# run-house/kubetorch

Hardware: NVIDIA H100
Metric: parallel_map_arg_plus_result_GBps (higher is better)
Workload: dtype f32

## Files before the change

### kubetorch_b200/csrc/ktb_map.cu

```cuda
#include "ktb_common.cuh"

#include <algorithm>
#include <atomic>

namespace ktb {

extern int g_red_ctas_per_sm;
extern int g_red_loads;
extern int g_red_fold;
extern int g_seg_large;
extern int g_mlp_chunk_rows;
}
extern int g_mlp_stage_ce;
namespace ktb {
extern std::atomic<int> g_host_zero_copy;
}
extern std::atomic<int> g_push_scatter_ctas_per_sm;
extern std::atomic<int> g_push_slice;
namespace ktb {

static std::atomic<int> g_vec_ctas_per_sm{0};
static std::atomic<int> g_tma_ctas_per_sm{1};
static std::atomic<int> g_tma_cfg{0};
static std::atomic<int> g_auto_variant{KTB_VARIANT_VEC};
static std::atomic<int> g_vec_flavor{2};
static std::atomic<int> g_vec_unroll{4};

constexpr int kVecThreads = 256;
constexpr int kVecUnroll = 4;
constexpr int kVecFlavor = 2;

template <int VB, int FL>
__device__ __forceinline__ void ld_vec(const uint8_t* p, uint32_t (&w)[VB / 4]) {
  static_assert(VB == 16, "sm_90 has no wider per-thread global access than 128 bits");
  if constexpr (FL == 1) {
    asm volatile("ld.global.v4.b32 {%0,%1,%2,%3}, [%4];"
                 : "=r"(w[0]), "=r"(w[1]), "=r"(w[2]), "=r"(w[3])
                 : "l"(p)
                 : "memory");
  } else if constexpr (FL == 2 || FL == 3) {
    ldg128_stream(p, w);
  } else {
    ldg128(p, w);
  }
}
template <int VB, int FL>
__device__ __forceinline__ void st_vec(uint8_t* p, const uint32_t (&w)[VB / 4]) {
  static_assert(VB == 16, "sm_90 has no wider per-thread global access than 128 bits");
  if constexpr (FL == 1) {
    asm volatile("st.global.v4.b32 [%0], {%1,%2,%3,%4};" ::"l"(p), "r"(w[0]), "r"(w[1]), "r"(w[2]), "r"(w[3])
                 : "memory");
  } else if constexpr (FL == 2) {
    stg128_stream(p, w);
  } else {
    stg128(p, w);
  }
}

template <int DT, int OP, int VB, int FL = kVecFlavor, int UNROLL = kVecUnroll>
__global__ void __launch_bounds__(kVecThreads)
    map_vec_kernel(const uint8_t* src, uint8_t* dst, size_t n_bytes, MapParams p) {
  constexpr int NW = VB / 4;
  constexpr int kVecUnroll = UNROLL;
  constexpr size_t TILE = (size_t)kVecThreads * kVecUnroll * VB;
  constexpr size_t ROW = (size_t)kVecThreads * VB;
  const size_t n_full = n_bytes / TILE;

  for (size_t t = blockIdx.x; t < n_full; t += gridDim.x) {
    const size_t off = t * TILE + (size_t)threadIdx.x * VB;
    uint32_t w[kVecUnroll][NW];
#pragma unroll
    for (int j = 0; j < kVecUnroll; ++j) ld_vec<VB, FL>(src + off + j * ROW, w[j]);
#pragma unroll
    for (int j = 0; j < kVecUnroll; ++j) {
      apply_words<DT, OP, NW>(w[j], p);
      st_vec<VB, FL>(dst + off + j * ROW, w[j]);
    }
  }

  if (blockIdx.x == (unsigned)(n_full % gridDim.x)) {
    const size_t base = n_full * TILE;
    const size_t n_vec = (n_bytes - base) / VB;
    for (size_t v = threadIdx.x; v < n_vec; v += kVecThreads) {
      uint32_t w[NW];
      ld_vec<VB, FL>(src + base + v * VB, w);
      apply_words<DT, OP, NW>(w, p);
      st_vec<VB, FL>(dst + base + v * VB, w);
    }
    constexpr size_t ES = (DT == KTB_U8) ? 1 : ((DT == KTB_BF16 || DT == KTB_F16) ? 2 : (DT == KTB_I64 ? 8 : 4));
    const size_t tail = base + n_vec * VB;
    const size_t n_tail = (n_bytes - tail) / ES;
    for (size_t e = threadIdx.x; e < n_tail; e += kVecThreads)
      apply_elem<DT, OP>(src + tail + e * ES, dst + tail + e * ES, p);
  }
}

template <int DT, int OP>
__global__ void __launch_bounds__(256)
    map_scalar_kernel(const uint8_t* src, uint8_t* dst, size_t n_elems, MapParams p) {
  constexpr size_t ES = (DT == KTB_U8) ? 1 : ((DT == KTB_BF16 || DT == KTB_F16) ? 2 : (DT == KTB_I64 ? 8 : 4));
  const size_t stride = (size_t)gridDim.x * blockDim.x;
  for (size_t i = (size_t)blockIdx.x * blockDim.x + threadIdx.x; i < n_elems; i += stride)
    apply_elem<DT, OP>(src + i * ES, dst + i * ES, p);
}

template <int DT, int OP, int STAGES, int STAGE_BYTES, int NT>
__global__ void __launch_bounds__(NT)
    map_tma_kernel(const uint8_t* src, uint8_t* dst, size_t n_bytes, MapParams p) {
  extern __shared__ __align__(128) uint8_t smem[];
  uint8_t* buf = smem;
  uint64_t* full = reinterpret_cast<uint64_t*>(smem + (size_t)STAGES * STAGE_BYTES);
  constexpr bool kCompute = !(OP == KTB_OP_IDENTITY || DT == KTB_U8);
// ... 13 lines not shown
#pragma unroll
    for (int s = 0; s < STAGES; ++s) mbar_init(&full[s], 1);
    fence_barrier_init();
    fence_proxy_async_smem();
  }
  __syncthreads();

  if (threadIdx.x == 0) {
    const size_t pre = my_n < (size_t)STAGES ? my_n : (size_t)STAGES;
    for (size_t k = 0; k < pre; ++k) {
      const uint32_t len = tile_len(k);
      mbar_expect_tx(&full[k], len);
      bulk_g2s(buf + k * STAGE_BYTES, src + tile_off(k), len, &full[k]);
    }
  }

  if (kCompute || threadIdx.x == 0) {
    for (size_t k = 0; k < my_n; ++k) {
      const int s = (int)(k % STAGES);
      const uint32_t parity = (uint32_t)((k / STAGES) & 1);
      const uint32_t len = tile_len(k);
      mbar_wait(&full[s], parity);
      if constexpr (kCompute) {
        uint4* tile = reinterpret_cast<uint4*>(buf + (size_t)s * STAGE_BYTES);
        const uint32_t nv = len >> 4;
        for (uint32_t v = threadIdx.x; v < nv; v += NT) {
          uint4 q = tile[v];
          uint32_t w[4] = {q.x, q.y, q.z, q.w};
          apply_words<DT, OP, 4>(w, p);
          tile[v] = make_uint4(w[0], w[1], w[2], w[3]);
        }
        fence_proxy_async_smem();
        __syncthreads();
      }
      if (threadIdx.x == 0) {
        bulk_s2g(dst + tile_off(k), buf + (size_t)s * STAGE_BYTES, len);
        bulk_commit();
        if (k >= 1 && (k - 1 + STAGES) < my_n) {
          bulk_wait_read<1>();
          const size_t kn = k - 1 + STAGES;
          const int sn = (int)((k - 1) % STAGES);
          const uint32_t ln = tile_len(kn);
          mbar_expect_tx(&full[sn], ln);
          bulk_g2s(buf + (size_t)sn * STAGE_BYTES, src + tile_off(kn), ln, &full[sn]);
        }
      }
    }
    if (threadIdx.x == 0) bulk_wait_all<0>();
  }

  if (blockIdx.x == 0) {
    constexpr size_t ES = (DT == KTB_U8) ? 1 : ((DT == KTB_BF16 || DT == KTB_F16) ? 2 : (DT == KTB_I64 ? 8 : 4));
    const size_t n_tail = (n_bytes - n16) / ES;
    for (size_t e = threadIdx.x; e < n_tail; e += NT)
      apply_elem<DT, OP>(src + n16 + e * ES, dst + n16 + e * ES, p);
  }
}

template <int DT, int OP>
static int launch_typed(int dev, const uint8_t* src, uint8_t* dst, size_t n_elems, size_t es,
                        const MapParams& p, int variant, cudaStream_t stream) {
  const DeviceInfo* di = device_info(dev);
  const size_t n_bytes = n_elems * es;
  const uintptr_t both = (uintptr_t)src | (uintptr_t)dst;

  if (variant == KTB_VARIANT_AUTO) variant = g_auto_variant.load();
  if (variant == KTB_VARIANT_TMA && (both & 15)) variant = KTB_VARIANT_VEC;
  if (variant == KTB_VARIANT_VEC && (both & 15)) variant = KTB_VARIANT_SCALAR;

  if (variant == KTB_VARIANT_VEC) {
    const int per_sm = g_vec_ctas_per_sm.load();
    auto grid_for = [&](size_t tile_bytes) {
      size_t tiles = std::max<size_t>(n_bytes / tile_bytes, 1);
      if (per_sm <= 0) return (int)std::min<size_t>(tiles, 0x7fffffffULL);
      return (int)std::min<size_t>(tiles, (size_t)di->sm_count * per_sm);
    };
    constexpr bool kTunable = (DT == KTB_U8) || (DT == KTB_F32 && OP == KTB_OP_SCALE);
    const int fl = kTunable ? g_vec_flavor.load() : kVecFlavor;
    const int un = kTunable ? g_vec_unroll.load() : kVecUnroll;
#define KTB_VEC16(FL, UN)                                                                          \
  map_vec_kernel<DT, OP, 16, FL, UN>                                                               \
      <<<grid_for((size_t)kVecThreads * (UN)*16), kVecThreads, 0, stream>>>(src, dst, n_bytes, p)
    if constexpr (kTunable) {
      if (un == 2) {
        if (fl == 1) KTB_VEC16(1, 2); else if (fl == 2) KTB_VEC16(2, 2); else if (fl == 3) KTB_VEC16(3, 2); else KTB_VEC16(0, 2);
      } else if (un == 8) {
        if (fl == 1) KTB_VEC16(1, 8); else if (fl == 2) KTB_VEC16(2, 8); else if (fl == 3) KTB_VEC16(3, 8); else KTB_VEC16(0, 8);
      } else {
        if (fl == 1) KTB_VEC16(1, 4); else if (fl == 2) KTB_VEC16(2, 4); else if (fl == 3) KTB_VEC16(3, 4); else KTB_VEC16(0, 4);
      }
    } else {
      (void)fl; (void)un;
      KTB_VEC16(kVecFlavor, kVecUnroll);
    }
#undef KTB_VEC16
  } else if (variant == KTB_VARIANT_TMA) {
    const int cfg = g_tma_cfg.load();
    const int per_sm = std::max(1, g_tma_ctas_per_sm.load());
#define KTB_LAUNCH_TMA(ST, SB, NT)                                                              \
  do {                                                                                          \
    constexpr size_t smem_bytes = (size_t)(ST) * (SB) + (ST) * sizeof(uint64_t);                \
    auto kfn = map_tma_kernel<DT, OP, ST, SB, NT>;                                              \
    KTB_CK(cudaFuncSetAttribute(kfn, cudaFuncAttributeMaxDynamicSharedMemorySize,               \
                                (int)smem_bytes));                                              \
    size_t tiles = ((n_bytes & ~(size_t)15) + (SB)-1) / (SB);                                   \
    int grid = (int)std::min<size_t>(std::max<size_t>(tiles, 1), (size_t)di->sm_count * per_sm); \
    kfn<<<grid, NT, smem_bytes, stream>>>(src, dst, n_bytes, p);                                \
  } while (0)
    if (cfg == 1) {
      KTB_LAUNCH_TMA(6, 32768, 256);
    } else if (cfg == 2) {
      KTB_LAUNCH_TMA(6, 16384, 256);
    } else if (cfg == 3) {
      KTB_LAUNCH_TMA(3, 65536, 512);
    } else {
      KTB_LAUNCH_TMA(4, 32768, 256);
    }
#undef KTB_LAUNCH_TMA
  } else if (variant == KTB_VARIANT_SCALAR) {
    size_t blocks = (n_elems + 255) / 256;
    int grid = (int)std::min<size_t>(std::max<size_t>(blocks, 1), (size_t)di->sm_count * 8);
    map_scalar_kernel<DT, OP><<<grid, 256, 0, stream>>>(src, dst, n_elems, p);
  } else {
    set_error("ktb_map: unknown variant %d", variant);
    return KTB_ERR_ARG;
  }
  KTB_CK(cudaGetLastError());
  return KTB_OK;
}

int launch_map(int dev, int op, int dtype, const void* src_, void* dst_, size_t n_elems,
               const MapParams& p, int variant, cudaStream_t stream) {
  const uint8_t* src = static_cast<const uint8_t*>(src_);
  uint8_t* dst = static_cast<uint8_t*>(dst_);
  const size_t es = dtype_size(dtype);
  KTB_REQUIRE(es != 0, KTB_ERR_ARG, "ktb_map: unknown dtype %d", dtype);
  KTB_REQUIRE(op >= KTB_OP_IDENTITY && op <= KTB_OP_AFFINE, KTB_ERR_ARG, "ktb_map: unknown op %d", op);
  KTB_REQUIRE(!(dtype == KTB_U8 && op != KTB_OP_IDENTITY), KTB_ERR_ARG,
              "ktb_map: KTB_U8 supports KTB_OP_IDENTITY only");
  if (n_elems == 0) return KTB_OK;
  KTB_REQUIRE(src && dst, KTB_ERR_ARG, "ktb_map: null src/dst with n_elems=%zu", n_elems);
  KTB_REQUIRE((((uintptr_t)src | (uintptr_t)dst) & (es - 1)) == 0, KTB_ERR_ARG,
              "ktb_map: src/dst not aligned to the element size %zu", es);
  KTB_REQUIRE(n_elems <= (SIZE_MAX / 8), KTB_ERR_ARG, "ktb_map: n_elems too large");
  if (src != dst) {
    const uint8_t* se = src + n_elems * es;
    const uint8_t* de = dst + n_elems * es;
    KTB_REQUIRE(se <= dst || de <= src, KTB_ERR_ARG, "ktb_map: src and dst partially overlap");
  }

  if (op == KTB_OP_IDENTITY)
    return launch_typed<KTB_U8, KTB_OP_IDENTITY>(dev, src, dst, n_elems * es, 1, p, variant, stream);

#define KTB_CASE(DT)                                                                              \
  case DT:                                                                                        \
    return (op == KTB_OP_SCALE)                                                                   \
               ? launch_typed<DT, KTB_OP_SCALE>(dev, src, dst, n_elems, es, p, variant, stream)   \
               : launch_typed<DT, KTB_OP_AFFINE>(dev, src, dst, n_elems, es, p, variant, stream);
  switch (dtype) {
    KTB_CASE(KTB_F32)
    KTB_CASE(KTB_BF16)
    KTB_CASE(KTB_I32)
    KTB_CASE(KTB_I64)
    KTB_CASE(KTB_F16)
  }
#undef KTB_CASE
  set_error("ktb_map: unsupported dtype/op %d/%d", dtype, op);
// ... 66 lines not shown
```

### kubetorch_b200/csrc/ktb_mlp.cu

```cuda
#include "ktb_common.cuh"

#include <cuda.h>
#include <algorithm>
#include <atomic>
#include <climits>
#include <cmath>
#include <mutex>

namespace ktb {

constexpr int kMlpBlockM = 128;
constexpr int kMlpBlockK = 64;
constexpr int kMlpWgmmaK = 16;
constexpr int kMlpStages = 4;
constexpr int kMlpConsumers = 256;
constexpr int kMlpThreads = kMlpConsumers + 32;
int g_mlp_chunk_rows = 16896;

__device__ __forceinline__ void tma_load_2d(void* smem_dst, const CUtensorMap* map, int c0, int c1, uint64_t* bar) {
  asm volatile(
      "cp.async.bulk.tensor.2d.shared::cluster.global.mbarrier::complete_tx::bytes [%0], [%1, {%3, %4}], [%2];" ::
          "r"(smem_u32(smem_dst)),
      "l"(map), "r"(smem_u32(bar)), "r"(c0), "r"(c1)
      : "memory");
}
__device__ __forceinline__ void prefetch_tensormap(const CUtensorMap* map) {
  asm volatile("prefetch.tensormap [%0];" ::"l"(map) : "memory");
}
__device__ __forceinline__ void mbar_arrive(uint64_t* bar) {
  asm volatile("mbarrier.arrive.shared::cta.b64 _, [%0];" ::"r"(smem_u32(bar)) : "memory");
}
__device__ __forceinline__ void wgmma_fence() { asm volatile("wgmma.fence.sync.aligned;" ::: "memory"); }
__device__ __forceinline__ void wgmma_commit() { asm volatile("wgmma.commit_group.sync.aligned;" ::: "memory"); }
__device__ __forceinline__ void wgmma_wait_all() { asm volatile("wgmma.wait_group.sync.aligned 0;" ::: "memory"); }

__device__ __forceinline__ uint64_t make_smem_desc_sw128(const void* smem_tile) {
  const uint32_t addr = smem_u32(smem_tile);
  uint64_t d = 0;
  d |= (uint64_t)((addr & 0x3FFFFu) >> 4);
  d |= (uint64_t)1 << 16;
  d |= (uint64_t)(1024u >> 4) << 32;
  d |= (uint64_t)1 << 62;
  return d;
}

template <int N>
struct Wgmma;
template <>
struct Wgmma<256> {
  __device__ __forceinline__ static void mma(float (&d)[128], uint64_t adesc, uint64_t bdesc, uint32_t scale_d) {
    asm volatile(
        "{\n"
        ".reg .pred p;\n"
        "setp.ne.b32 p, %130, 0;\n"
        "wgmma.mma_async.sync.aligned.m64n256k16.f32.bf16.bf16 "
        "{%0,%1,%2,%3,%4,%5,%6,%7,%8,%9,%10,%11,%12,%13,%14,%15,%16,%17,%18,%19,%20,%21,%22,%23,%24,%25,%26,%27,%28,%29,%30,%31,%32,%33,%34,%35,%36,%37,%38,%39,%40,%41,%42,%43,%44,%45,%46,%47,%48,%49,%50,%51,%52,%53,%54,%55,%56,%57,%58,%59,%60,%61,%62,%63,%64,%65,%66,%67,%68,%69,%70,%71,%72,%73,%74,%75,%76,%77,%78,%79,%80,%81,%82,%83,%84,%85,%86,%87,%88,%89,%90,%91,%92,%93,%94,%95,%96,%97,%98,%99,%100,%101,%102,%103,%104,%105,%106,%107,%108,%109,%110,%111,%112,%113,%114,%115,%116,%117,%118,%119,%120,%121,%122,%123,%124,%125,%126,%127}, "
        "%128, %129, p, 1, 1, 0, 0;\n"
        "}\n"
        : "+f"(d[0]), "+f"(d[1]), "+f"(d[2]), "+f"(d[3]), "+f"(d[4]), "+f"(d[5]), "+f"(d[6]), "+f"(d[7]), "+f"(d[8]), "+f"(d[9]), "+f"(d[10]), "+f"(d[11]), "+f"(d[12]), "+f"(d[13]), "+f"(d[14]), "+f"(d[15]), "+f"(d[16]), "+f"(d[17]), "+f"(d[18]), "+f"(d[19]), "+f"(d[20]), "+f"(d[21]), "+f"(d[22]), "+f"(d[23]), "+f"(d[24]), "+f"(d[25]), "+f"(d[26]), "+f"(d[27]), "+f"(d[28]), "+f"(d[29]), "+f"(d[30]), "+f"(d[31]), "+f"(d[32]), "+f"(d[33]), "+f"(d[34]), "+f"(d[35]), "+f"(d[36]), "+f"(d[37]), "+f"(d[38]), "+f"(d[39]), "+f"(d[40]), "+f"(d[41]), "+f"(d[42]), "+f"(d[43]), "+f"(d[44]), "+f"(d[45]), "+f"(d[46]), "+f"(d[47]), "+f"(d[48]), "+f"(d[49]), "+f"(d[50]), "+f"(d[51]), "+f"(d[52]), "+f"(d[53]), "+f"(d[54]), "+f"(d[55]), "+f"(d[56]), "+f"(d[57]), "+f"(d[58]), "+f"(d[59]), "+f"(d[60]), "+f"(d[61]), "+f"(d[62]), "+f"(d[63]), "+f"(d[64]), "+f"(d[65]), "+f"(d[66]), "+f"(d[67]), "+f"(d[68]), "+f"(d[69]), "+f"(d[70]), "+f"(d[71]), "+f"(d[72]), "+f"(d[73]), "+f"(d[74]), "+f"(d[75]), "+f"(d[76]), "+f"(d[77]), "+f"(d[78]), "+f"(d[79]), "+f"(d[80]), "+f"(d[81]), "+f"(d[82]), "+f"(d[83]), "+f"(d[84]), "+f"(d[85]), "+f"(d[86]), "+f"(d[87]), "+f"(d[88]), "+f"(d[89]), "+f"(d[90]), "+f"(d[91]), "+f"(d[92]), "+f"(d[93]), "+f"(d[94]), "+f"(d[95]), "+f"(d[96]), "+f"(d[97]), "+f"(d[98]), "+f"(d[99]), "+f"(d[100]), "+f"(d[101]), "+f"(d[102]), "+f"(d[103]), "+f"(d[104]), "+f"(d[105]), "+f"(d[106]), "+f"(d[107]), "+f"(d[108]), "+f"(d[109]), "+f"(d[110]), "+f"(d[111]), "+f"(d[112]), "+f"(d[113]), "+f"(d[114]), "+f"(d[115]), "+f"(d[116]), "+f"(d[117]), "+f"(d[118]), "+f"(d[119]), "+f"(d[120]), "+f"(d[121]), "+f"(d[122]), "+f"(d[123]), "+f"(d[124]), "+f"(d[125]), "+f"(d[126]), "+f"(d[127])
        : "l"(adesc), "l"(bdesc), "r"(scale_d));
  }
};

template <>
struct Wgmma<128> {
  __device__ __forceinline__ static void mma(float (&d)[64], uint64_t adesc, uint64_t bdesc, uint32_t scale_d) {
    asm volatile(
        "{\n"
        ".reg .pred p;\n"
        "setp.ne.b32 p, %66, 0;\n"
        "wgmma.mma_async.sync.aligned.m64n128k16.f32.bf16.bf16 "
        "{%0,%1,%2,%3,%4,%5,%6,%7,%8,%9,%10,%11,%12,%13,%14,%15,%16,%17,%18,%19,%20,%21,%22,%23,%24,%25,%26,%27,%28,%29,%30,%31,%32,%33,%34,%35,%36,%37,%38,%39,%40,%41,%42,%43,%44,%45,%46,%47,%48,%49,%50,%51,%52,%53,%54,%55,%56,%57,%58,%59,%60,%61,%62,%63}, "
        "%64, %65, p, 1, 1, 0, 0;\n"
        "}\n"
        : "+f"(d[0]), "+f"(d[1]), "+f"(d[2]), "+f"(d[3]), "+f"(d[4]), "+f"(d[5]), "+f"(d[6]), "+f"(d[7]), "+f"(d[8]), "+f"(d[9]), "+f"(d[10]), "+f"(d[11]), "+f"(d[12]), "+f"(d[13]), "+f"(d[14]), "+f"(d[15]), "+f"(d[16]), "+f"(d[17]), "+f"(d[18]), "+f"(d[19]), "+f"(d[20]), "+f"(d[21]), "+f"(d[22]), "+f"(d[23]), "+f"(d[24]), "+f"(d[25]), "+f"(d[26]), "+f"(d[27]), "+f"(d[28]), "+f"(d[29]), "+f"(d[30]), "+f"(d[31]), "+f"(d[32]), "+f"(d[33]), "+f"(d[34]), "+f"(d[35]), "+f"(d[36]), "+f"(d[37]), "+f"(d[38]), "+f"(d[39]), "+f"(d[40]), "+f"(d[41]), "+f"(d[42]), "+f"(d[43]), "+f"(d[44]), "+f"(d[45]), "+f"(d[46]), "+f"(d[47]), "+f"(d[48]), "+f"(d[49]), "+f"(d[50]), "+f"(d[51]), "+f"(d[52]), "+f"(d[53]), "+f"(d[54]), "+f"(d[55]), "+f"(d[56]), "+f"(d[57]), "+f"(d[58]), "+f"(d[59]), "+f"(d[60]), "+f"(d[61]), "+f"(d[62]), "+f"(d[63])
        : "l"(adesc), "l"(bdesc), "r"(scale_d));
  }
};

template <>
struct Wgmma<64> {
  __device__ __forceinline__ static void mma(float (&d)[32], uint64_t adesc, uint64_t bdesc, uint32_t scale_d) {
    asm volatile(
        "{\n"
        ".reg .pred p;\n"
        "setp.ne.b32 p, %34, 0;\n"
        "wgmma.mma_async.sync.aligned.m64n64k16.f32.bf16.bf16 "
        "{%0,%1,%2,%3,%4,%5,%6,%7,%8,%9,%10,%11,%12,%13,%14,%15,%16,%17,%18,%19,%20,%21,%22,%23,%24,%25,%26,%27,%28,%29,%30,%31}, "
        "%32, %33, p, 1, 1, 0, 0;\n"
        "}\n"
        : "+f"(d[0]), "+f"(d[1]), "+f"(d[2]), "+f"(d[3]), "+f"(d[4]), "+f"(d[5]), "+f"(d[6]), "+f"(d[7]), "+f"(d[8]), "+f"(d[9]), "+f"(d[10]), "+f"(d[11]), "+f"(d[12]), "+f"(d[13]), "+f"(d[14]), "+f"(d[15]), "+f"(d[16]), "+f"(d[17]), "+f"(d[18]), "+f"(d[19]), "+f"(d[20]), "+f"(d[21]), "+f"(d[22]), "+f"(d[23]), "+f"(d[24]), "+f"(d[25]), "+f"(d[26]), "+f"(d[27]), "+f"(d[28]), "+f"(d[29]), "+f"(d[30]), "+f"(d[31])
        : "l"(adesc), "l"(bdesc), "r"(scale_d));
  }
};
template <int BLOCK_N, int STAGES>
struct MlpSmem {
  static constexpr int kABytes = kMlpBlockM * kMlpBlockK * 2;
  static constexpr int kBBytes = BLOCK_N * kMlpBlockK * 2;
  static constexpr int kStageBytes = kABytes + kBBytes;
  static constexpr int kBarrierOff = STAGES * kStageBytes;
  static constexpr int kTotal = kBarrierOff + 2 * STAGES * 8 + 1024 ;
};

template <int BLOCK_N, int STAGES>
__device__ __forceinline__ bool mlp_tile_mainloop(const CUtensorMap* map_a, const CUtensorMap* map_b, int K, int m0,
                                                  int n0, float (&acc)[BLOCK_N / 2]) {
  using S = MlpSmem<BLOCK_N, STAGES>;
  extern __shared__ uint8_t smem_raw[];
  uint8_t* smem = reinterpret_cast<uint8_t*>((reinterpret_cast<uintptr_t>(smem_raw) + 1023) & ~(uintptr_t)1023);
  uint64_t* full = reinterpret_cast<uint64_t*>(smem + S::kBarrierOff);
  uint64_t* empty = full + STAGES;

  const int warp = threadIdx.x >> 5;
  const int lane = threadIdx.x & 31;
  const int num_kb = K / kMlpBlockK;

  if (threadIdx.x == 0) {
#pragma unroll
    for (int s = 0; s < STAGES; ++s) {
      mbar_init(&full[s], 1);
      mbar_init(&empty[s], kMlpConsumers);
    }
    fence_barrier_init();
  }
  __syncthreads();

  if (warp == kMlpConsumers / 32) {
    if (lane == 0) {
      prefetch_tensormap(map_a);
      prefetch_tensormap(map_b);
      for (int kb = 0; kb < num_kb; ++kb) {
        const int s = kb % STAGES;
        mbar_wait(&empty[s], ((kb / STAGES) & 1) ^ 1);
        uint8_t* a_dst = smem + (size_t)s * S::kStageBytes;
        mbar_expect_tx(&full[s], S::kStageBytes);
        tma_load_2d(a_dst, map_a, kb * kMlpBlockK, m0, &full[s]);
        tma_load_2d(a_dst + S::kABytes, map_b, kb * kMlpBlockK, n0, &full[s]);
      }
    }
    return false;
  }

  const int wg = warp >> 2;
#pragma unroll
  for (int i = 0; i < BLOCK_N / 2; ++i) acc[i] = 0.f;
  for (int kb = 0; kb < num_kb; ++kb) {
    const int s = kb % STAGES;
    mbar_wait(&full[s], (kb / STAGES) & 1);
    const uint8_t* a_src = smem + (size_t)s * S::kStageBytes + wg * 64 * 128;
    const uint64_t adesc = make_smem_desc_sw128(a_src);
    const uint64_t bdesc = make_smem_desc_sw128(smem + (size_t)s * S::kStageBytes + S::kABytes);
    wgmma_fence();
#pragma unroll
    for (int k = 0; k < kMlpBlockK / kMlpWgmmaK; ++k) {
      Wgmma<BLOCK_N>::mma(acc, adesc + (uint64_t)(2 * k), bdesc + (uint64_t)(2 * k), (uint32_t)((kb | k) != 0));
    }
    wgmma_commit();
    wgmma_wait_all();
    mbar_arrive(&empty[s]);
  }
  return true;
}

__device__ __forceinline__ bool argmax_before(float v, int col, float best, int best_col) {
  const bool v_nan = v != v, best_nan = best != best;
  if (v_nan || best_nan) return v_nan && (!best_nan || col < best_col);
  return v > best || (v == best && col < best_col);
}

__device__ __forceinline__ uint4 philox4x32_10(uint4 c, uint2 k) {
#pragma unroll
  for (int i = 0; i < 10; ++i) {
    const uint32_t hi0 = __umulhi(0xD2511F53u, c.x), lo0 = 0xD2511F53u * c.x;
    const uint32_t hi1 = __umulhi(0xCD9E8D57u, c.z), lo1 = 0xCD9E8D57u * c.z;
    c = make_uint4(hi1 ^ c.y ^ k.x, lo1, hi0 ^ c.w ^ k.y, lo0);
    k.x += 0x9E3779B9u;
    k.y += 0xBB67AE85u;
  }
  return c;
}

__device__ __forceinline__ float gumbel_of(uint32_t x) {
  const float u = (float)(2u * (x >> 9) + 1u) * 5.9604644775390625e-8f;
  return -logf(-logf(u));
}

__device__ __forceinline__ void layer_pair(float a0, float a1, float a2, float a3, const __nv_bfloat16* bias, int col,
                                           int n_valid, int relu, __nv_bfloat162& y0, __nv_bfloat162& y1) {
  float v[4] = {a0, a1, a2, a3};
  if (bias != nullptr) {
#pragma unroll
    for (int c = 0; c < 2; ++c) {
      if (col + c < n_valid) {
        const float b = __bfloat162float(bias[col + c]);
        v[c] += b;
        v[2 + c] += b;
      }
    }
  }
  if (relu) {
#pragma unroll
    for (int q = 0; q < 4; ++q) v[q] = fmaxf(v[q], 0.f);
  }
  y0 = __floats2bfloat162_rn(v[0], v[1]);
  y1 = __floats2bfloat162_rn(v[2], v[3]);
}

template <int BLOCK_N>
__device__ __forceinline__ void sample_epilogue(const float (&acc)[BLOCK_N / 2], const __nv_bfloat16* bias, int col0,
                                                int n_valid, int relu, int row, bool st0, bool st1, int64_t* actions,
                                                float* log_probs, uint64_t seed, uint64_t row_base) {
  float mx[2] = {-INFINITY, -INFINITY};
  __nv_bfloat162 y[BLOCK_N / 4];
#pragma unroll
  for (int j = 0; j < BLOCK_N / 8; ++j) {
    const int col = col0 + 8 * j;
    if (col >= n_valid) continue;
    layer_pair(acc[4 * j], acc[4 * j + 1], acc[4 * j + 2], acc[4 * j + 3], bias, col, n_valid, relu, y[2 * j],
               y[2 * j + 1]);
#pragma unroll
    for (int q = 0; q < 4; ++q) {
      const float v = q & 1 ? __high2float(y[2 * j + (q >> 1)]) : __low2float(y[2 * j + (q >> 1)]);
      if (col + (q & 1) < n_valid && v > mx[q >> 1]) mx[q >> 1] = v;
    }
  }
#pragma unroll
  for (int h = 0; h < 2; ++h) {
#pragma unroll
    for (int m = 1; m <= 2; m <<= 1) {
      const float o = __shfl_xor_sync(0xffffffffu, mx[h], m);
      if (o > mx[h]) mx[h] = o;
    }
  }
  const uint2 key = make_uint2((uint32_t)seed, (uint32_t)(seed >> 32));
  float best[2] = {-INFINITY, -INFINITY}, best_y[2] = {0.f, 0.f}, sum[2] = {0.f, 0.f};
  int best_col[2] = {INT_MAX, INT_MAX};
#pragma unroll
  for (int j = 0; j < BLOCK_N / 8; ++j) {
    const int col = col0 + 8 * j;
    if (col >= n_valid) continue;
#pragma unroll
    for (int h = 0; h < 2; ++h) {
      const uint64_t i = row_base + (uint64_t)(row + 8 * h);
      const uint4 x = philox4x32_10(make_uint4((uint32_t)i, (uint32_t)(i >> 32), (uint32_t)col >> 1, 0u), key);
#pragma unroll
      for (int c = 0; c < 2; ++c) {
        if (col + c >= n_valid) continue;
        const float v = c ? __high2float(y[2 * j + h]) : __low2float(y[2 * j + h]);
        const float s = v + gumbel_of(c ? x.y : x.x);
        if (argmax_before(s, col + c, best[h], best_col[h])) {
          best[h] = s;
          best_col[h] = col + c;
          best_y[h] = v;
        }
        sum[h] += v == mx[h] ? 1.f : expf(v - mx[h]);
      }
    }
  }
#pragma unroll
  for (int h = 0; h < 2; ++h) {
#pragma unroll
    for (int m = 1; m <= 2; m <<= 1) {
      const float ov = __shfl_xor_sync(0xffffffffu, best[h], m);
      const int oc = __shfl_xor_sync(0xffffffffu, best_col[h], m);
      const float oy = __shfl_xor_sync(0xffffffffu, best_y[h], m);
      sum[h] += __shfl_xor_sync(0xffffffffu, sum[h], m);
      if (argmax_before(ov, oc, best[h], best_col[h])) {
        best[h] = ov;
        best_col[h] = oc;
        best_y[h] = oy;
      }
    }
  }
  if ((threadIdx.x & 3) == 0) {
    if (st0) {
      actions[row] = best_col[0];
      log_probs[row] = best_y[0] - mx[0] - logf(sum[0]);
    }
    if (st1) {
      actions[row + 8] = best_col[1];
      log_probs[row + 8] = best_y[1] - mx[1] - logf(sum[1]);
    }
  }
}

template <int BLOCK_N, int STAGES>
__device__ __forceinline__ void gaussian_epilogue(const float (&acc)[BLOCK_N / 2], const __nv_bfloat16* bias, int col0,
                                                  int n_valid, int relu, int row, bool st0, bool st1,
                                                  const float* log_std, float* actions, float* log_probs,
                                                  uint64_t seed, uint64_t row_base) {
  asm volatile("" : "+l"(seed), "+l"(row_base), "+l"(bias), "+r"(col0), "+r"(n_valid), "+r"(row));
  using S = MlpSmem<BLOCK_N, STAGES>;
  static_assert(BLOCK_N / 64 <= STAGES, "each warp's bf16 pairs fill its 16 A rows of BLOCK_N / 64 stages");
  extern __shared__ uint8_t smem_raw[];
  uint8_t* smem = reinterpret_cast<uint8_t*>((reinterpret_cast<uintptr_t>(smem_raw) + 1023) & ~(uintptr_t)1023);
  uint8_t* mine = smem + (threadIdx.x >> 5) * 16 * 128 + (threadIdx.x & 31) * 4;
  auto slot = [&](int w) { return reinterpret_cast<__nv_bfloat162*>(mine + (w >> 4) * S::kStageBytes + (w & 15) * 128); };
#pragma unroll
  for (int j = 0; j < BLOCK_N / 8; ++j) {
    const int col = col0 + 8 * j;
    if (col >= n_valid) continue;
    layer_pair(acc[4 * j], acc[4 * j + 1], acc[4 * j + 2], acc[4 * j + 3], bias, col, n_valid, relu, *slot(2 * j),
               *slot(2 * j + 1));
  }
  const uint2 key = make_uint2((uint32_t)seed, (uint32_t)(seed >> 32));
  const bool pairs = (n_valid & 1) == 0 && ((uintptr_t)actions & 7) == 0;
  float sum[2] = {0.f, 0.f};
#pragma unroll 1
  for (int j = 0; j < BLOCK_N / 8; ++j) {
    const int col = col0 + 8 * j;
    if (col >= n_valid) break;
    const __nv_bfloat162 y[2] = {*slot(2 * j), *slot(2 * j + 1)};
    const bool has1 = col + 1 < n_valid;
    const float ls[2] = {log_std[col], has1 ? log_std[col + 1] : 0.f};
    const float sg[2] = {expf(ls[0]), expf(ls[1])};
#pragma unroll
    for (int h = 0; h < 2; ++h) {
      const uint64_t i = row_base + (uint64_t)(row + 8 * h);
      const uint4 x = philox4x32_10(make_uint4((uint32_t)i, (uint32_t)(i >> 32), (uint32_t)col >> 1, 1u), key);
      float a[2];
#pragma unroll
      for (int c = 0; c < 2; ++c) {
        const float u = (float)(2u * ((c ? x.y : x.x) >> 9) + 1u) * 5.9604644775390625e-8f;
        const float z = normcdfinvf(u);
        a[c] = __fadd_rn(c ? __high2float(y[h]) : __low2float(y[h]), __fmul_rn(sg[c], z));
        if (c == 0 || has1) sum[h] += 0.5f * z * z + ls[c];
      }
      if (!(h ? st1 : st0)) continue;
      float* p = actions + (size_t)(row + 8 * h) * n_valid + col;
      if (pairs) {
        *reinterpret_cast<float2*>(p) = make_float2(a[0], a[1]);
      } else {
        p[0] = a[0];
        if (has1) p[1] = a[1];
      }
    }
  }
#pragma unroll
  for (int h = 0; h < 2; ++h) {
#pragma unroll
    for (int m = 1; m <= 2; m <<= 1) sum[h] += __shfl_xor_sync(0xffffffffu, sum[h], m);
  }
  if ((threadIdx.x & 3) == 0) {
    const float c = (float)n_valid * 0.918938533204672742f;
    if (st0) log_probs[row] = -sum[0] - c;
    if (st1) log_probs[row + 8] = -sum[1] - c;
  }
}

template <int BLOCK_N, int STAGES>
__global__ void __launch_bounds__(kMlpThreads, 1)
    mlp_layer_wgmma_kernel(const __grid_constant__ CUtensorMap map_a, const __grid_constant__ CUtensorMap map_b,
                           const __nv_bfloat16* __restrict__ bias, __nv_bfloat16* __restrict__ C,
                           int64_t* __restrict__ actions, float* __restrict__ log_probs, uint64_t seed,
                           uint64_t row_base, const float* __restrict__ log_std, float* __restrict__ gauss_actions,
                           int ldc, int n_valid, int K, int rows, int relu) {
  const int n0 = blockIdx.x * BLOCK_N;
  const int m0 = blockIdx.y * kMlpBlockM;
  const int lane = threadIdx.x & 31;
  const int col0 = n0 + 2 * (lane & 3);
  float acc[BLOCK_N / 2];
  if (!mlp_tile_mainloop<BLOCK_N, STAGES>(&map_a, &map_b, K, m0, n0, acc)) return;
  const int warp = threadIdx.x >> 5;
  const int wg = warp >> 2;

  const int row = m0 + wg * 64 + (warp & 3) * 16 + (lane >> 2);
  const bool st0 = row < rows, st1 = row + 8 < rows;
  if (log_std != nullptr) {
    gaussian_epilogue<BLOCK_N, STAGES>(acc, bias, col0, n_valid, relu, row, st0, st1, log_std, gauss_actions,
                                       log_probs, seed, row_base);
    return;
  }
  if (log_probs != nullptr) {
    sample_epilogue<BLOCK_N>(acc, bias, col0, n_valid, relu, row, st0, st1, actions, log_probs, seed, row_base);
    return;
  }
  const bool pairs = C != nullptr && (ldc & 1) == 0 && ((uintptr_t)C & 3) == 0;
  if (pairs && actions == nullptr && n0 + BLOCK_N <= n_valid) {
    __nv_bfloat16* p0 = C + (size_t)row * ldc + col0;
    __nv_bfloat16* p1 = p0 + (size_t)8 * ldc;
#pragma unroll
    for (int j = 0; j < BLOCK_N / 8; ++j) {
      __nv_bfloat162 y0, y1;
      layer_pair(acc[4 * j], acc[4 * j + 1], acc[4 * j + 2], acc[4 * j + 3], bias, col0 + 8 * j, n_valid, relu, y0, y1);
      if (st0) *reinterpret_cast<__nv_bfloat162*>(p0 + 8 * j) = y0;
      if (st1) *reinterpret_cast<__nv_bfloat162*>(p1 + 8 * j) = y1;
    }
    return;
  }
  float best[2] = {-INFINITY, -INFINITY};
  int best_col[2] = {INT_MAX, INT_MAX};
#pragma unroll
  for (int j = 0; j < BLOCK_N / 8; ++j) {
    const int col = col0 + 8 * j;
    __nv_bfloat162 y0, y1;
    layer_pair(acc[4 * j], acc[4 * j + 1], acc[4 * j + 2], acc[4 * j + 3], bias, col, n_valid, relu, y0, y1);
    if (C != nullptr) {
      __nv_bfloat16* p0 = C + (size_t)row * ldc + col;
      __nv_bfloat16* p1 = p0 + (size_t)8 * ldc;
      if (pairs && col + 1 < n_valid) {
        if (st0) *reinterpret_cast<__nv_bfloat162*>(p0) = y0;
        if (st1) *reinterpret_cast<__nv_bfloat162*>(p1) = y1;
      } else {
        if (st0 && col < n_valid) p0[0] = y0.x;
        if (st1 && col < n_valid) p1[0] = y1.x;
        if (st0 && col + 1 < n_valid) p0[1] = y0.y;
        if (st1 && col + 1 < n_valid) p1[1] = y1.y;
      }
    }
    if (actions != nullptr) {
      const float r[4] = {__low2float(y0), __high2float(y0), __low2float(y1), __high2float(y1)};
#pragma unroll
      for (int q = 0; q < 4; ++q) {
        const int h = q >> 1, c = col + (q & 1);
        if (c < n_valid && argmax_before(r[q], c, best[h], best_col[h])) {
          best[h] = r[q];
          best_col[h] = c;
        }
      }
    }
  }
  if (actions != nullptr) {
#pragma unroll
    for (int h = 0; h < 2; ++h) {
#pragma unroll
      for (int m = 1; m <= 2; m <<= 1) {
        const float ov = __shfl_xor_sync(0xffffffffu, best[h], m);
        const int oc = __shfl_xor_sync(0xffffffffu, best_col[h], m);
        if (argmax_before(ov, oc, best[h], best_col[h])) {
          best[h] = ov;
          best_col[h] = oc;
        }
      }
    }
    if ((lane & 3) == 0) {
      if (st0) actions[row] = best_col[0];
      if (st1) actions[row + 8] = best_col[1];
    }
  }
}

typedef CUresult (*PFN_tensorMapEncodeTiled)(CUtensorMap*, CUtensorMapDataType, cuuint32_t, void*, const cuuint64_t*,
                                             const cuuint64_t*, const cuuint32_t*, const cuuint32_t*,
                                             CUtensorMapInterleave, CUtensorMapSwizzle, CUtensorMapL2promotion,
                                             CUtensorMapFloatOOBfill);
static PFN_tensorMapEncodeTiled g_encode = nullptr;
static std::once_flag g_encode_once;

static int get_encoder() {
  std::call_once(g_encode_once, [] {
    void* fn = nullptr;
    cudaDriverEntryPointQueryResult qres;
    if (cudaGetDriverEntryPoint("cuTensorMapEncodeTiled", &fn, cudaEnableDefault, &qres) == cudaSuccess &&
        qres == cudaDriverEntryPointSuccess)
      g_encode = reinterpret_cast<PFN_tensorMapEncodeTiled>(fn);
  });
  KTB_REQUIRE(g_encode != nullptr, KTB_ERR_CUDA, "cuTensorMapEncodeTiled is not available from the driver");
  return KTB_OK;
}

static int encode_map(CUtensorMap* map, const void* base, uint64_t rows, uint64_t cols, uint32_t box_rows);

static int make_map(CUtensorMap* map, const void* base, uint64_t rows, uint64_t cols, uint32_t box_rows) {
  struct Key {
    const void* base;
    uint64_t rows, cols;
    uint32_t box;
    bool operator==(const Key& o) const { return base == o.base && rows == o.rows && cols == o.cols && box == o.box; }
  };
  struct Slot {
    Key key;
    CUtensorMap map;
    bool used = false;
  };
  constexpr int kSlots = 64;
  thread_local Slot cache[kSlots];
  const Key k{base, rows, cols, box_rows};
  const size_t h = ((uintptr_t)base >> 8) * 0x9E3779B97F4A7C15ull + rows * 31 + cols * 7 + box_rows;
  Slot& s = cache[h % kSlots];
  if (s.used && s.key == k) {
    *map = s.map;
    return KTB_OK;
  }
  int rc = encode_map(map, base, rows, cols, box_rows);
  if (rc) return rc;
  s.key = k;
  s.map = *map;
  s.used = true;
  return KTB_OK;
}

static int encode_map(CUtensorMap* map, const void* base, uint64_t rows, uint64_t cols, uint32_t box_rows) {
  cuuint64_t gdim[2] = {cols, rows};
  cuuint64_t gstride[1] = {cols * 2};
  cuuint32_t box[2] = {(cuuint32_t)kMlpBlockK, box_rows};
  cuuint32_t estr[2] = {1, 1};
  CUresult r = g_encode(map, CU_TENSOR_MAP_DATA_TYPE_BFLOAT16, 2, const_cast<void*>(base), gdim, gstride, box, estr,
                        CU_TENSOR_MAP_INTERLEAVE_NONE, CU_TENSOR_MAP_SWIZZLE_128B, CU_TENSOR_MAP_L2_PROMOTION_L2_256B,
                        CU_TENSOR_MAP_FLOAT_OOB_FILL_NONE);
  KTB_REQUIRE(r == CUDA_SUCCESS, KTB_ERR_CUDA, "cuTensorMapEncodeTiled failed with CUresult %d", (int)r);
  return KTB_OK;
}

template <typename KernelT>
static int ensure_smem_attr(KernelT kfn, int smem_bytes, std::atomic<unsigned>& done_mask, int dev) {
  if (dev >= 0 && dev < 32 && (done_mask.load(std::memory_order_acquire) & (1u << dev))) return KTB_OK;
  cudaError_t e = cudaFuncSetAttribute(kfn, cudaFuncAttributeMaxDynamicSharedMemorySize, smem_bytes);
  if (e != cudaSuccess) {
    set_error("cudaFuncSetAttribute(max dynamic shared memory = %d) failed: %s", smem_bytes, cudaGetErrorString(e));
    return KTB_ERR_CUDA;
  }
  if (dev >= 0 && dev < 32) done_mask.fetch_or(1u << dev, std::memory_order_release);
  return KTB_OK;
}

enum class HeadKind {
  kGreedy,
  kSample,
  kGaussian,
};

struct HeadOut {
  void* logits = nullptr;
  int64_t* actions = nullptr;
  float* log_probs = nullptr;
  uint64_t seed = 0, row_base = 0;
  const float* log_std = nullptr;
  float* gauss_actions = nullptr;

  HeadOut from_row(size_t r0, int d_out) const {
    HeadOut h = *this;
    if (logits) h.logits = static_cast<__nv_bfloat16*>(logits) + r0 * d_out;
    if (actions) h.actions += r0;
    if (log_probs) h.log_probs += r0;
    if (gauss_actions) h.gauss_actions += r0 * d_out;
    h.row_base += r0;
    return h;
  }
};

template <int BLOCK_N>
static int launch_layer(int dev, const void* A, const void* B, const void* bias, void* C, const HeadOut& head,
                        size_t M, int N, int K, int ldc, bool relu, cudaStream_t stream) {
  using S = MlpSmem<BLOCK_N, kMlpStages>;
  static_assert(S::kTotal <= 232448, "the TMA ring must fit the 227 KiB a block may own");
  CUtensorMap ma, mb;
  int rc = make_map(&ma, A, M, (uint64_t)K, kMlpBlockM);
  if (rc) return rc;
  rc = make_map(&mb, B, (uint64_t)N, (uint64_t)K, BLOCK_N);
  if (rc) return rc;
  auto kfn = mlp_layer_wgmma_kernel<BLOCK_N, kMlpStages>;
  static std::atomic<unsigned> attr_done{0};
  rc = ensure_smem_attr(kfn, S::kTotal, attr_done, dev);
  if (rc) return rc;
  dim3 grid((unsigned)((N + BLOCK_N - 1) / BLOCK_N), (unsigned)((M + kMlpBlockM - 1) / kMlpBlockM));
  kfn<<<grid, kMlpThreads, S::kTotal, stream>>>(ma, mb, static_cast<const __nv_bfloat16*>(bias),
                                                static_cast<__nv_bfloat16*>(C), head.actions, head.log_probs,
                                                head.seed, head.row_base, head.log_std, head.gauss_actions, ldc, N, K,
                                                (int)M, relu);
  KTB_CK(cudaGetLastError());
  return KTB_OK;
}

struct MlpParams {
  const void *W1, *b1, *W2, *b2, *W3, *b3;
  HeadKind kind;
  HeadOut out;
};

static int mlp_chunk(int dev, const MlpParams& p, const void* a1, void* h1, void* h2, size_t r0, size_t rows, int d_in,
                     int d_hidden, int d_out, cudaEvent_t consumed, cudaStream_t st) {
  int rc = launch_layer<256>(dev, a1, p.W1, p.b1, h1, HeadOut{}, rows, d_hidden, d_in, d_hidden, true, st);
  if (rc) return rc;
  if (consumed) KTB_CK(cudaEventRecord(consumed, st));
  rc = launch_layer<256>(dev, h1, p.W2, p.b2, h2, HeadOut{}, rows, d_hidden, d_hidden, d_hidden, true, st);
  if (rc) return rc;
  const HeadOut h = p.out.from_row(r0, d_out);
  const auto head = d_out <= 64 ? launch_layer<64> : d_out <= 128 ? launch_layer<128> : launch_layer<256>;
  return head(dev, h2, p.W3, p.b3, h.logits, h, rows, d_out, d_hidden, d_out, false, st);
}

static int mlp_check(const char* fn, size_t M, int d_in, int d_hidden, int d_out, const MlpParams& p, const void* obs,
                     const void* scratch, const void* stage) {
  KTB_REQUIRE(d_in > 0 && d_in % kMlpBlockK == 0, KTB_ERR_ARG, "%s: d_in=%d must be a multiple of 64", fn, d_in);
  KTB_REQUIRE(d_hidden > 0 && d_hidden % 256 == 0, KTB_ERR_ARG, "%s: d_hidden=%d must be a multiple of 256", fn,
              d_hidden);
  if (M > 0) {
    const HeadOut& o = p.out;
    switch (p.kind) {
      case HeadKind::kGreedy:
        KTB_REQUIRE(o.logits || o.actions, KTB_ERR_ARG, "%s: logits and actions are both null", fn);
        break;
      case HeadKind::kSample:
        KTB_REQUIRE(o.actions && o.log_probs, KTB_ERR_ARG, "%s: actions and log_probs are required", fn);
        break;
      case HeadKind::kGaussian:
        KTB_REQUIRE(o.log_std && o.gauss_actions && o.log_probs, KTB_ERR_ARG,
                    "%s: log_std, actions and log_probs are required", fn);
        KTB_REQUIRE((((uintptr_t)o.log_std | (uintptr_t)o.gauss_actions) & 3) == 0, KTB_ERR_ARG,
                    "%s: log_std and actions must be 4-byte aligned", fn);
        break;
    }
    KTB_REQUIRE(d_out >= 1, KTB_ERR_ARG, "%s: d_out=%d must be positive", fn, d_out);
    KTB_REQUIRE(d_out <= 256, KTB_ERR_UNSUPPORTED, "%s: d_out=%d (heads up to 256 wide)", fn, d_out);
    KTB_REQUIRE((((uintptr_t)o.logits | (uintptr_t)p.b1 | (uintptr_t)p.b2 | (uintptr_t)p.b3) & 1) == 0, KTB_ERR_ARG,
                "%s: logits and biases must be 2-byte aligned", fn);
    KTB_REQUIRE(((uintptr_t)o.actions & 7) == 0, KTB_ERR_ARG, "%s: actions must be 8-byte aligned", fn);
    KTB_REQUIRE(((uintptr_t)o.log_probs & 3) == 0, KTB_ERR_ARG, "%s: log_probs must be 4-byte aligned", fn);
  }
  KTB_REQUIRE((((uintptr_t)obs | (uintptr_t)p.W1 | (uintptr_t)p.W2 | (uintptr_t)p.W3 | (uintptr_t)scratch |
                (uintptr_t)stage) & 15) == 0,
              KTB_ERR_ARG, "%s: obs, weights, scratch and stage must be 16-byte aligned", fn);
  return KTB_OK;
}
}

using namespace ktb;

extern "C" {

size_t ktb_mlp_scratch_bytes(size_t M, int d_hidden) {
  const size_t rows = std::min<size_t>(M, (size_t)g_mlp_chunk_rows);
  return 2 * rows * (size_t)d_hidden * 2;
}

size_t ktb_mlp_stage_bytes(size_t M, int d_in) {
  const size_t rows = std::min<size_t>(M, (size_t)g_mlp_chunk_rows);
  return 2 * rows * (size_t)d_in * 2;
}

int g_mlp_stage_ce = 0;

static int mlp_run(const char* fn, int dev, const void* obs, size_t M, int d_in, int d_hidden, int d_out,
                   const MlpParams& p, void* scratch, void* stage, uintptr_t stream) {
  int rc = require_device(dev);
  if (rc) return rc;
  if (M == 0) return KTB_OK;
  KTB_REQUIRE(obs && p.W1 && p.W2 && p.W3 && scratch, KTB_ERR_ARG, "%s: null argument", fn);
// ... 207 lines not shown
```

Before: 2939.

## Use unroll-1 vector map kernel and make MLP GEMM persistent with async wgmma waits

The map kernel's default vector unroll drops from 4 to 1, so each thread handles one 16-byte chunk and the grid holds more CTAs. Separately, the MLP layer kernel becomes persistent: a grid sized by occupancy loops over tiles, the producer keeps the TMA ring running across tiles, and consumers wait on all but one wgmma group so a stage is released one step later. These are two unrelated changes. The map change affects the measured map bandwidth and trades loop overhead for more CTA scheduling; the MLP change targets launch overhead and TMA/MMA overlap.

```diff
diff --git a/kubetorch_b200/csrc/ktb_map.cu b/kubetorch_b200/csrc/ktb_map.cu
--- a/kubetorch_b200/csrc/ktb_map.cu
+++ b/kubetorch_b200/csrc/ktb_map.cu
@@ -24,10 +24,10 @@
 static std::atomic<int> g_tma_cfg{0};
 static std::atomic<int> g_auto_variant{KTB_VARIANT_VEC};
 static std::atomic<int> g_vec_flavor{2};
-static std::atomic<int> g_vec_unroll{4};
+static std::atomic<int> g_vec_unroll{1};
 
 constexpr int kVecThreads = 256;
-constexpr int kVecUnroll = 4;
+constexpr int kVecUnroll = 1;
 constexpr int kVecFlavor = 2;
 
 template <int VB, int FL>
@@ -207,7 +207,9 @@
   map_vec_kernel<DT, OP, 16, FL, UN>                                                               \
       <<<grid_for((size_t)kVecThreads * (UN)*16), kVecThreads, 0, stream>>>(src, dst, n_bytes, p)
     if constexpr (kTunable) {
-      if (un == 2) {
+      if (un == 1) {
+        if (fl == 1) KTB_VEC16(1, 1); else if (fl == 2) KTB_VEC16(2, 1); else if (fl == 3) KTB_VEC16(3, 1); else KTB_VEC16(0, 1);
+      } else if (un == 2) {
         if (fl == 1) KTB_VEC16(1, 2); else if (fl == 2) KTB_VEC16(2, 2); else if (fl == 3) KTB_VEC16(3, 2); else KTB_VEC16(0, 2);
       } else if (un == 8) {
         if (fl == 1) KTB_VEC16(1, 8); else if (fl == 2) KTB_VEC16(2, 8); else if (fl == 3) KTB_VEC16(3, 8); else KTB_VEC16(0, 8);
diff --git a/kubetorch_b200/csrc/ktb_mlp.cu b/kubetorch_b200/csrc/ktb_mlp.cu
--- a/kubetorch_b200/csrc/ktb_mlp.cu
+++ b/kubetorch_b200/csrc/ktb_mlp.cu
@@ -32,7 +32,8 @@
 }
 __device__ __forceinline__ void wgmma_fence() { asm volatile("wgmma.fence.sync.aligned;" ::: "memory"); }
 __device__ __forceinline__ void wgmma_commit() { asm volatile("wgmma.commit_group.sync.aligned;" ::: "memory"); }
-__device__ __forceinline__ void wgmma_wait_all() { asm volatile("wgmma.wait_group.sync.aligned 0;" ::: "memory"); }
+template <int N>
+__device__ __forceinline__ void wgmma_wait() { asm volatile("wgmma.wait_group.sync.aligned %0;" ::"n"(N) : "memory"); }
 
 __device__ __forceinline__ uint64_t make_smem_desc_sw128(const void* smem_tile) {
   const uint32_t addr = smem_u32(smem_tile);
@@ -103,50 +104,54 @@
 };
 
 template <int BLOCK_N, int STAGES>
-__device__ __forceinline__ bool mlp_tile_mainloop(const CUtensorMap* map_a, const CUtensorMap* map_b, int K, int m0,
-                                                  int n0, float (&acc)[BLOCK_N / 2]) {
+__device__ __forceinline__ uint8_t* mlp_ring() {
+  extern __shared__ uint8_t smem_raw[];
+  return reinterpret_cast<uint8_t*>((reinterpret_cast<uintptr_t>(smem_raw) + 1023) & ~(uintptr_t)1023);
+}
+
+struct MlpTile {
+  int m0, n0;
+};
+template <int BLOCK_N>
+__device__ __forceinline__ MlpTile mlp_tile(int t, int tiles_n) {
+  return MlpTile{(t / tiles_n) * kMlpBlockM, (t % tiles_n) * BLOCK_N};
+}
+
+template <int BLOCK_N, int STAGES>
+__device__ __forceinline__ void mlp_producer(const CUtensorMap* map_a, const CUtensorMap* map_b, int num_kb, int tiles,
+                                             int tiles_n) {
   using S = MlpSmem<BLOCK_N, STAGES>;
-  extern __shared__ uint8_t smem_raw[];
-  uint8_t* smem = reinterpret_cast<uint8_t*>((reinterpret_cast<uintptr_t>(smem_raw) + 1023) & ~(uintptr_t)1023);
+  uint8_t* smem = mlp_ring<BLOCK_N, STAGES>();
   uint64_t* full = reinterpret_cast<uint64_t*>(smem + S::kBarrierOff);
   uint64_t* empty = full + STAGES;
-
-  const int warp = threadIdx.x >> 5;
-  const int lane = threadIdx.x & 31;
-  const int num_kb = K / kMlpBlockK;
-
-  if (threadIdx.x == 0) {
-#pragma unroll
-    for (int s = 0; s < STAGES; ++s) {
-      mbar_init(&full[s], 1);
-      mbar_init(&empty[s], kMlpConsumers);
-    }
-    fence_barrier_init();
-  }
-  __syncthreads();
-
-  if (warp == kMlpConsumers / 32) {
-    if (lane == 0) {
-      prefetch_tensormap(map_a);
-      prefetch_tensormap(map_b);
-      for (int kb = 0; kb < num_kb; ++kb) {
-        const int s = kb % STAGES;
-        mbar_wait(&empty[s], ((kb / STAGES) & 1) ^ 1);
-        uint8_t* a_dst = smem + (size_t)s * S::kStageBytes;
-        mbar_expect_tx(&full[s], S::kStageBytes);
-        tma_load_2d(a_dst, map_a, kb * kMlpBlockK, m0, &full[s]);
-        tma_load_2d(a_dst + S::kABytes, map_b, kb * kMlpBlockK, n0, &full[s]);
-      }
-    }
-    return false;
-  }
-
-  const int wg = warp >> 2;
+  prefetch_tensormap(map_a);
+  prefetch_tensormap(map_b);
+  int it = 0;
+  for (int t = blockIdx.x; t < tiles; t += gridDim.x) {
+    const MlpTile tile = mlp_tile<BLOCK_N>(t, tiles_n);
+    for (int kb = 0; kb < num_kb; ++kb, ++it) {
+      const int s = it % STAGES;
+      mbar_wait(&empty[s], ((it / STAGES) & 1) ^ 1);
+      uint8_t* a_dst = smem + (size_t)s * S::kStageBytes;
+      mbar_expect_tx(&full[s], S::kStageBytes);
+      tma_load_2d(a_dst, map_a, kb * kMlpBlockK, tile.m0, &full[s]);
+      tma_load_2d(a_dst + S::kABytes, map_b, kb * kMlpBlockK, tile.n0, &full[s]);
+    }
+  }
+}
+
+template <int BLOCK_N, int STAGES>
+__device__ __forceinline__ void mlp_tile_mma(int num_kb, int held, int& it, float (&acc)[BLOCK_N / 2]) {
+  using S = MlpSmem<BLOCK_N, STAGES>;
+  const uint8_t* smem = mlp_ring<BLOCK_N, STAGES>();
+  uint64_t* full = reinterpret_cast<uint64_t*>(mlp_ring<BLOCK_N, STAGES>() + S::kBarrierOff);
+  uint64_t* empty = full + STAGES;
+  const int wg = threadIdx.x >> 7;
 #pragma unroll
   for (int i = 0; i < BLOCK_N / 2; ++i) acc[i] = 0.f;
-  for (int kb = 0; kb < num_kb; ++kb) {
-    const int s = kb % STAGES;
-    mbar_wait(&full[s], (kb / STAGES) & 1);
+  for (int kb = 0; kb < num_kb; ++kb, ++it) {
+    const int s = it % STAGES;
+    mbar_wait(&full[s], (it / STAGES) & 1);
     const uint8_t* a_src = smem + (size_t)s * S::kStageBytes + wg * 64 * 128;
     const uint64_t adesc = make_smem_desc_sw128(a_src);
     const uint64_t bdesc = make_smem_desc_sw128(smem + (size_t)s * S::kStageBytes + S::kABytes);
@@ -156,10 +161,18 @@
       Wgmma<BLOCK_N>::mma(acc, adesc + (uint64_t)(2 * k), bdesc + (uint64_t)(2 * k), (uint32_t)((kb | k) != 0));
     }
     wgmma_commit();
-    wgmma_wait_all();
-    mbar_arrive(&empty[s]);
-  }
-  return true;
+    wgmma_wait<1>();
+    if (kb > 0 && kb <= num_kb - held) mbar_arrive(&empty[(it - 1) % STAGES]);
+  }
+  wgmma_wait<0>();
+  if (held == 0) mbar_arrive(&empty[(it - 1) % STAGES]);
+}
+
+template <int BLOCK_N, int STAGES>
+__device__ __forceinline__ void mlp_release(int held, int it) {
+  using S = MlpSmem<BLOCK_N, STAGES>;
+  uint64_t* empty = reinterpret_cast<uint64_t*>(mlp_ring<BLOCK_N, STAGES>() + S::kBarrierOff) + STAGES;
+  for (int j = it - held; j < it; ++j) mbar_arrive(&empty[j % STAGES]);
 }
 
 __device__ __forceinline__ bool argmax_before(float v, int col, float best, int best_col) {
@@ -211,7 +224,7 @@
                                                 int n_valid, int relu, int row, bool st0, bool st1, int64_t* actions,
                                                 float* log_probs, uint64_t seed, uint64_t row_base) {
   float mx[2] = {-INFINITY, -INFINITY};
-  __nv_bfloat162 y[BLOCK_N / 4];
+  __nv_bfloat162 y[BLOCK_N / 4] = {};
 #pragma unroll
   for (int j = 0; j < BLOCK_N / 8; ++j) {
     const int col = col0 + 8 * j;
@@ -349,18 +362,15 @@
 }
 
 template <int BLOCK_N, int STAGES>
-__global__ void __launch_bounds__(kMlpThreads, 1)
-    mlp_layer_wgmma_kernel(const __grid_constant__ CUtensorMap map_a, const __grid_constant__ CUtensorMap map_b,
-                           const __nv_bfloat16* __restrict__ bias, __nv_bfloat16* __restrict__ C,
-                           int64_t* __restrict__ actions, float* __restrict__ log_probs, uint64_t seed,
-                           uint64_t row_base, const float* __restrict__ log_std, float* __restrict__ gauss_actions,
-                           int ldc, int n_valid, int K, int rows, int relu) {
-  const int n0 = blockIdx.x * BLOCK_N;
-  const int m0 = blockIdx.y * kMlpBlockM;
+__device__ __forceinline__ void mlp_tile_epilogue(const float (&acc)[BLOCK_N / 2], int m0, int n0,
+                                                  const __nv_bfloat16* __restrict__ bias,
+                                                  __nv_bfloat16* __restrict__ C, int64_t* __restrict__ actions,
+                                                  float* __restrict__ log_probs, uint64_t seed, uint64_t row_base,
+                                                  const float* __restrict__ log_std,
+                                                  float* __restrict__ gauss_actions, int ldc, int n_valid, int rows,
+                                                  int relu) {
   const int lane = threadIdx.x & 31;
   const int col0 = n0 + 2 * (lane & 3);
-  float acc[BLOCK_N / 2];
-  if (!mlp_tile_mainloop<BLOCK_N, STAGES>(&map_a, &map_b, K, m0, n0, acc)) return;
   const int warp = threadIdx.x >> 5;
   const int wg = warp >> 2;
 
@@ -372,6 +382,7 @@
     return;
   }
   if (log_probs != nullptr) {
+    asm volatile("" : "+l"(seed));
     sample_epilogue<BLOCK_N>(acc, bias, col0, n_valid, relu, row, st0, st1, actions, log_probs, seed, row_base);
     return;
   }
@@ -436,6 +447,49 @@
     if ((lane & 3) == 0) {
       if (st0) actions[row] = best_col[0];
       if (st1) actions[row + 8] = best_col[1];
+    }
+  }
+}
+
+template <int BLOCK_N, int STAGES>
+__global__ void __launch_bounds__(kMlpThreads, 1)
+    mlp_layer_wgmma_kernel(const __grid_constant__ CUtensorMap map_a, const __grid_constant__ CUtensorMap map_b,
+                           const __nv_bfloat16* __restrict__ bias, __nv_bfloat16* __restrict__ C,
+                           int64_t* __restrict__ actions, float* __restrict__ log_probs, uint64_t seed,
+                           uint64_t row_base, const float* __restrict__ log_std, float* __restrict__ gauss_actions,
+                           int ldc, int n_valid, int K, int rows, int relu) {
+  using S = MlpSmem<BLOCK_N, STAGES>;
+  uint64_t* full = reinterpret_cast<uint64_t*>(mlp_ring<BLOCK_N, STAGES>() + S::kBarrierOff);
+  uint64_t* empty = full + STAGES;
+  if (threadIdx.x == 0) {
+#pragma unroll
+    for (int s = 0; s < STAGES; ++s) {
+      mbar_init(&full[s], 1);
+      mbar_init(&empty[s], kMlpConsumers);
+    }
+    fence_barrier_init();
+  }
+  __syncthreads();
+
+  const int num_kb = K / kMlpBlockK;
+  const int tiles_n = (n_valid + BLOCK_N - 1) / BLOCK_N;
+  const int tiles = tiles_n * ((rows + kMlpBlockM - 1) / kMlpBlockM);
+  if (threadIdx.x >> 5 == kMlpConsumers / 32) {
+    if ((threadIdx.x & 31) == 0) mlp_producer<BLOCK_N, STAGES>(&map_a, &map_b, num_kb, tiles, tiles_n);
+    return;
+  }
+  const int held = log_std != nullptr ? min(num_kb, STAGES) : 0;
+  int it = 0;
+#pragma unroll 1
+  for (int t = blockIdx.x; t < tiles; t += gridDim.x) {
+    const MlpTile tile = mlp_tile<BLOCK_N>(t, tiles_n);
+    float acc[BLOCK_N / 2];
+    mlp_tile_mma<BLOCK_N, STAGES>(num_kb, held, it, acc);
+    mlp_tile_epilogue<BLOCK_N, STAGES>(acc, tile.m0, tile.n0, bias, C, actions, log_probs, seed, row_base, log_std,
+                                       gauss_actions, ldc, n_valid, rows, relu);
+    if (held) {
+      fence_proxy_async_smem();
+      mlp_release<BLOCK_N, STAGES>(held, it);
     }
   }
 }
@@ -514,6 +568,21 @@
   return KTB_OK;
 }
 
+template <typename KernelT>
+static int resident_ctas(KernelT kfn, int smem_bytes, std::atomic<int> (&per_sm)[kMaxDevices], int dev, int* out) {
+  int n = per_sm[dev].load(std::memory_order_relaxed);
+  if (n == 0) {
+    cudaError_t e = cudaOccupancyMaxActiveBlocksPerMultiprocessor(&n, kfn, kMlpThreads, smem_bytes);
+    if (e != cudaSuccess || n < 1) {
+      set_error("cudaOccupancyMaxActiveBlocksPerMultiprocessor gave %d CTAs per SM: %s", n, cudaGetErrorString(e));
+      return KTB_ERR_CUDA;
+    }
+    per_sm[dev].store(n, std::memory_order_relaxed);
+  }
+  *out = n;
+  return KTB_OK;
+}
+
 enum class HeadKind {
   kGreedy,
   kSample,
@@ -553,7 +622,12 @@
   static std::atomic<unsigned> attr_done{0};
   rc = ensure_smem_attr(kfn, S::kTotal, attr_done, dev);
   if (rc) return rc;
-  dim3 grid((unsigned)((N + BLOCK_N - 1) / BLOCK_N), (unsigned)((M + kMlpBlockM - 1) / kMlpBlockM));
+  static std::atomic<int> per_sm[kMaxDevices];
+  int resident = 0;
+  rc = resident_ctas(kfn, S::kTotal, per_sm, dev, &resident);
+  if (rc) return rc;
+  const size_t tiles = (size_t)((N + BLOCK_N - 1) / BLOCK_N) * ((M + kMlpBlockM - 1) / kMlpBlockM);
+  const unsigned grid = (unsigned)std::min<size_t>(tiles, (size_t)device_info(dev)->sm_count * resident);
   kfn<<<grid, kMlpThreads, S::kTotal, stream>>>(ma, mb, static_cast<const __nv_bfloat16*>(bias),
                                                 static_cast<__nv_bfloat16*>(C), head.actions, head.log_probs,
                                                 head.seed, head.row_base, head.log_std, head.gauss_actions, ldc, N, K,
```

New measurement: 2973 (median of 6 runs). 1.01x the previous value.
